# evroon/mav-detection

Measured on AMD Instinct MI355X. Metric: frame-pairs/sec at 1920x1080, higher is better.
Workload: dtype f32; 1 GPU; 1920x1080, batch 64 per GPU, Farneback + FoE + phi/threshold + box; global_batch=64, parallelism=frame-parallel x1, record_exchange=none (1 GPU), torch_in_process=False

## Files before the change

mav-detection_amd/csrc/kernels_flow.hip:

```cpp
#include "mavflow_internal.h"

#include <algorithm>
#include <type_traits>

static __device__ __forceinline__ int clampi(int v, int lo, int hi) { return v < lo ? lo : (v > hi ? hi : v); }

struct TileMap { int tiles_x, tiles_y, per_img, n_tiles, strip_w, xcd, ty0; };
static __device__ __forceinline__ bool tile_of_block(const TileMap& tm, int* s, int* tx, int* ty)
{
    const int per = ((int)gridDim.x + 7) >> 3;
    const int tile = tm.xcd ? (int)(blockIdx.x & 7) * per + (int)(blockIdx.x >> 3) : (int)blockIdx.x;
    if (tile >= tm.n_tiles) return false;
    const int img = tile / tm.per_img;
    int tr = tile - img * tm.per_img;
    const int strip_tiles = tm.strip_w * tm.tiles_y;
    const int st = tr / strip_tiles;
    tr -= st * strip_tiles;
    const int x_base = st * tm.strip_w;
    const int sw = min(tm.strip_w, tm.tiles_x - x_base);
    const int row = tr / sw;
    *s = img; *ty = row + tm.ty0; *tx = x_base + tr - row * sw;
    return true;
}
static TileMap make_tile_map(int w, int h, int G, int tile_w, int tile_h, int ty0 = 0, int ty1 = -1, int strip = 0)
// ... 758 lines not shown
    const int dword_ok = quad_ok(f);
    const int esize = (int)sizeof(T);
    if (f.G <= 8) return blur_multi_launch(st, f, dword_ok, jobs);
    bool done[MAV_MAX_JOBS] = {false};
    for (int i = 0; i < jobs.n; i++) {
        if (done[i]) continue;
        auto path_of = [&](const BlurJob& J) {
            if (J.w == f.W && J.h == f.H) return -1;
            const FusedPlan fp = fused_plan(f.W, f.H, J.w, J.h, J.bp, dword_ok, esize);
            return fused_path_of(J.bp, fp.pitch_w, dword_ok, esize);
        };
        const int p = path_of(jobs.j[i]);
        BlurJobs sub{0, 0, {}};
        for (int k = i; k < jobs.n; k++)
            if (!done[k] && path_of(jobs.j[k]) == p) { sub.j[sub.n++] = jobs.j[k]; done[k] = true; }
        blur_multi_launch(st, f, dword_ok, sub);
    }
}

template <typename T>
__global__ __launch_bounds__(256) void k_blur3(const T* __restrict__ img, const T* __restrict__ img2, int split,
                                               size_t img_stride, int W, int H, float* __restrict__ out, size_t out_stride)
{
    blur3_block(image_of(img, img2, split, img_stride, blockIdx.z), out + (size_t)blockIdx.z * out_stride, W, H, blockIdx.x, blockIdx.y);
}

template <typename T>
bool blur_resize_needs_tmp(const FrameRun<T>& f, const LayerTarget& t)
{
    return !blur3_fast_ok(f.runs(), t) && !blur_resize_is_fused(f.W, f.H, t.w, t.h, t.bp.ksize, (int)sizeof(T));
}
template <typename T>
void launch_blur_resize(hipStream_t st, const FrameRun<T>& frames, const LayerTarget& t, const BlurScratch& scratch)
{
    const FrameRun<T> f = frames.runs();
    const int G = f.G, W = f.W, H = f.H, w = t.w, h = t.h;
    const BlurParams& bp = t.bp;
    if (blur3_fast_ok(f, t)) {
        dim3 grid((W / 4 + 63) / 64, ((H + 3) / 4 + 3) / 4, G);
        hipLaunchKernelGGL(k_blur3<T>, grid, dim3(256), 0, st, f.img, f.img2, f.split, f.img_stride, W, H, t.out, t.out_stride);
        return;
    }
    const int dword_ok = quad_ok(f);
    const int esize = (int)sizeof(T);
    const int pitch_w = staged_pitch_words(W, w, bp.ksize);
    if (!scratch.two_pass && blur_resize_is_fused(W, H, w, h, bp.ksize, esize)) {
        const FusedPlan fp = fused_plan(W, H, w, h, bp, dword_ok, esize);
        const dim3 grid((w + 63) / 64, (h + fp.th - 1) / fp.th, G);
        with_fused_path<T>(fused_path_of(bp, fp.pitch_w, dword_ok, esize), [&](auto P) {
            if constexpr (decltype(P)::value != FP_ANY)
                hipLaunchKernelGGL((k_blur_resize_fused<T, decltype(P)::value>), grid, dim3(256), fp.lds, st, f.img, f.img2, f.split, f.img_stride,
                                   W, H, w, h, bp, t.out, t.out_stride, fp.rows, fp.pitch_w, dword_ok, fp.th);
        });
        return;
    }
    int rows_blk = 16;
    while (rows_blk > 4 && (size_t)rows_blk * pitch_w * 4 * esize > 48 * 1024) rows_blk >>= 1;
    if ((size_t)rows_blk * pitch_w * 4 * esize <= 48 * 1024)
    {
        const int gx = (w + 63) / 64, nby = (H + rows_blk - 1) / rows_blk;
        const int gy = nby;
        const size_t lds_h = (size_t)((rows_blk * pitch_w * esize + 1) & ~1) * 4 + (size_t)((bp.ksize + 4) & ~3) * 8;
        hipLaunchKernelGGL(k_blur_resize_h<T>, dim3(gx, gy, G), dim3(256), lds_h, st, f.img, f.img2, f.split, f.img_stride, W, H, w, bp,
                           scratch.tmp, scratch.stride, rows_blk, pitch_w, dword_ok);
    }
    else
        hipLaunchKernelGGL(k_blur_resize_h_direct<T>, dim3((w + 63) / 64, ((H + 3) / 4 + 3) / 4, G), dim3(256), 0, st, f.img, f.img2, f.split,
                           f.img_stride, W, H, w, bp, scratch.tmp, scratch.stride);
    hipLaunchKernelGGL(k_blur_resize_v, dim3((w + 63) / 64, (h + 3) / 4, G), dim3(256), 0, st, (const float*)scratch.tmp, scratch.stride, H, w,
                       h, bp, t.out, t.out_stride);
}
#define MAV_BLUR_DEPTH(T)                                                                                     \
    template bool blur_multi_ok<T>(const FrameRun<T>&, const LayerTarget&);                                   \
    template void launch_blur_multi<T>(hipStream_t, const FrameRun<T>&, BlurJobs);                            \
    template bool blur_resize_needs_tmp<T>(const FrameRun<T>&, const LayerTarget&);                           \
    template void launch_blur_resize<T>(hipStream_t, const FrameRun<T>&, const LayerTarget&, const BlurScratch&);
MAV_BLUR_DEPTH(uint8_t)
MAV_BLUR_DEPTH(uint16_t)
MAV_BLUR_DEPTH(float)
#undef MAV_BLUR_DEPTH

#define PX 64
#define PY 16
template <int N_T>
static __device__ __forceinline__ void polyexp_tile(const float* __restrict__ src, float* __restrict__ dst, int w, int h, const PolyCoef& pc,
                                                    int tile_x, int tile_y, float* __restrict__ smem)
{
    const int n = N_T > 0 ? N_T : pc.n;
    const int EX = PX + 2 * n, EY = PY + 2 * n;
    float* tile = smem;
    float* v0 = tile + EX * EY;
    float* v1 = v0 + PY * EX;
    float* v2 = v1 + PY * EX;
    const int tid = threadIdx.x;
    const int x0 = tile_x * PX, y0 = tile_y * PY;

    if constexpr (N_T > 0) {
        constexpr int TOT = (PX + 2 * N_T) * (PY + 2 * N_T), CNT = (TOT + 255) / 256;
        float v[CNT];
#pragma unroll
        for (int j = 0; j < CNT; j++) {
            const int i = tid + 256 * j;
            if (i < TOT) {
                const int ly = i / EX, lx = i - ly * EX;
                const int gx = clampi(x0 - n + lx, 0, w - 1), gy = clampi(y0 - n + ly, 0, h - 1);
                v[j] = src[(size_t)gy * w + gx];
            }
        }
#pragma unroll
        for (int j = 0; j < CNT; j++)
            if (tid + 256 * j < TOT) tile[tid + 256 * j] = v[j];
    } else {
        for (int i = tid; i < EX * EY; i += 256) {
            const int ly = i / EX, lx = i - ly * EX;
            const int gx = clampi(x0 - n + lx, 0, w - 1), gy = clampi(y0 - n + ly, 0, h - 1);
            tile[i] = src[(size_t)gy * w + gx];
        }
    }
    __syncthreads();
    for (int i = tid; i < PY * EX; i += 256) {
        const int ly = i / EX, lx = i - ly * EX;
        const float* c = tile + (ly + n) * EX + lx;
        float t0 = c[0] * pc.g[0], t1 = 0.f, t2 = 0.f;
#pragma unroll
        for (int k = 1; k <= n; k++) {
            const float a = c[-k * EX], b = c[k * EX];
            const float p = a + b;
            t0 = fmaf(pc.g[k], p, t0);
            t1 = fmaf(pc.xg[k], b - a, t1);
            t2 = fmaf(pc.xxg[k], p, t2);
        }
        v0[i] = t0; v1[i] = t1; v2[i] = t2;
    }
    __syncthreads();
    const size_t npx = (size_t)w * h;
    for (int i = tid; i < PY * PX; i += 256) {
        const int ly = i >> 6, lx = i & 63;
        const int gx = x0 + lx, gy = y0 + ly;
        if (gx >= w || gy >= h) continue;
        const float* p0 = v0 + ly * EX + lx + n;
        const float* p1 = v1 + ly * EX + lx + n;
        const float* p2 = v2 + ly * EX + lx + n;
        float b1 = p0[0] * pc.g[0], b2 = 0.f, b3 = p1[0] * pc.g[0], b4 = 0.f, b5 = p2[0] * pc.g[0], b6 = 0.f;
#pragma unroll
        for (int k = 1; k <= n; k++) {
            const float a0 = p0[-k], c0 = p0[k], a1 = p1[-k], c1 = p1[k], a2 = p2[-k], c2 = p2[k];
            const float tg = c0 + a0;
            b1 = fmaf(tg, pc.g[k], b1);
            b4 = fmaf(tg, pc.xxg[k], b4);
            b2 = fmaf(c0 - a0, pc.xg[k], b2);
            b3 = fmaf(c1 + a1, pc.g[k], b3);
            b6 = fmaf(c1 - a1, pc.xg[k], b6);
            b5 = fmaf(c2 + a2, pc.g[k], b5);
        }
        const size_t o = (size_t)gy * w + gx;
        dst[o] = b3 * pc.ig11;
        dst[npx + o] = b2 * pc.ig11;
        dst[2 * npx + o] = fmaf(b5, pc.ig33, b1 * pc.ig03);
        dst[3 * npx + o] = fmaf(b4, pc.ig33, b1 * pc.ig03);
        dst[4 * npx + o] = b6 * pc.ig55;
    }
}

template <int N_T>
__global__ __launch_bounds__(256) void k_polyexp(const float* __restrict__ I, size_t I_stride, int w, int h, PolyCoef pc, TileMap tm,
                                                 float* __restrict__ R, size_t R_stride)
{
    int img_s, tile_x, tile_y;
    if (!tile_of_block(tm, &img_s, &tile_x, &tile_y)) return;
    extern __shared__ __attribute__((aligned(16))) float smem[];
    polyexp_tile<N_T>(I + (size_t)img_s * I_stride, R + (size_t)img_s * R_stride, w, h, pc, tile_x, tile_y, smem);
}

template <int N_T>
__global__ __launch_bounds__(256) void k_polyexp_multi(PolyJobs jobs, PolyCoef pc)
{
    int k = 0;
    for (int i = 1; i < jobs.n; i++) k = (int)blockIdx.x >= jobs.j[i].first_block ? i : k;
    const PolyJob J = jobs.j[k];
    const int tile = (int)blockIdx.x - J.first_block;
    const int img_s = tile / J.per_img, rem = tile - img_s * J.per_img;
    const int tile_y = rem / J.tiles_x, tile_x = rem - tile_y * J.tiles_x;
    extern __shared__ __attribute__((aligned(16))) float smem[];
    polyexp_tile<N_T>(J.I + (size_t)img_s * J.I_stride, J.R + (size_t)img_s * J.R_stride, J.w, J.h, pc, tile_x, tile_y, smem);
}
void launch_polyexp_multi(hipStream_t st, PolyJobs jobs, int G, const PolyCoef& pc)
{
    const int n = pc.n;
    const size_t lds = sizeof(float) * ((size_t)(PX + 2 * n) * (PY + 2 * n) + 3 * (size_t)PY * (PX + 2 * n));
    int blocks = 0;
    for (int i = 0; i < jobs.n; i++) {
        PolyJob& J = jobs.j[i];
        J.tiles_x = (J.w + PX - 1) / PX;
        J.per_img = J.tiles_x * ((J.h + PY - 1) / PY);
        J.first_block = blocks;
        blocks += J.per_img * G;
    }
    if (n == 8) hipLaunchKernelGGL(k_polyexp_multi<8>, dim3(blocks), dim3(256), lds, st, jobs, pc);
    else if (n == 7) hipLaunchKernelGGL(k_polyexp_multi<7>, dim3(blocks), dim3(256), lds, st, jobs, pc);
    else if (n == 5) hipLaunchKernelGGL(k_polyexp_multi<5>, dim3(blocks), dim3(256), lds, st, jobs, pc);
    else hipLaunchKernelGGL(k_polyexp_multi<0>, dim3(blocks), dim3(256), lds, st, jobs, pc);
}

void launch_polyexp(hipStream_t st, const float* I, size_t I_stride, int G, int w, int h, const PolyCoef& pc, float* R,
                    size_t R_stride)
{
    const int n = pc.n;
    const size_t lds = sizeof(float) * ((size_t)(PX + 2 * n) * (PY + 2 * n) + 3 * (size_t)PY * (PX + 2 * n));
    TileMap tm = make_tile_map(w, h, G, PX, PY);
    tm.xcd = 0;
    const dim3 grid(tile_grid(tm));
    if (n == 8)
        hipLaunchKernelGGL(k_polyexp<8>, grid, dim3(256), lds, st, I, I_stride, w, h, pc, tm, R, R_stride);
    else if (n == 7)
        hipLaunchKernelGGL(k_polyexp<7>, grid, dim3(256), lds, st, I, I_stride, w, h, pc, tm, R, R_stride);
    else if (n == 5)
        hipLaunchKernelGGL(k_polyexp<5>, grid, dim3(256), lds, st, I, I_stride, w, h, pc, tm, R, R_stride);
    else
        hipLaunchKernelGGL(k_polyexp<0>, grid, dim3(256), lds, st, I, I_stride, w, h, pc, tm, R, R_stride);
}

struct GatherPx {
    float p00[5], p01[5], p10[5], p11[5];
    float fx, fy;
    bool inside;
};
static __device__ __forceinline__ void gather_issue(const float* __restrict__ R1p, size_t npx, int w, int h, int x, int y, float dx,
                                                    float dy, GatherPx& g)
{
    float fx = x + dx, fy = y + dy;
    const int x1 = (int)floorf(fx), y1 = (int)floorf(fy);
    g.fx = fx - x1; g.fy = fy - y1;
    g.inside = (unsigned)x1 < (unsigned)(w - 1) && (unsigned)y1 < (unsigned)(h - 1);
    const int xc = g.inside ? x1 : 0, yc = g.inside ? y1 : 0;
    const float* p = R1p + (size_t)yc * w + xc;
#pragma unroll
    for (int c = 0; c < 5; c++) {
        g.p00[c] = p[0]; g.p01[c] = p[1]; g.p10[c] = p[w]; g.p11[c] = p[w + 1];
        p += npx;
    }
}
static __device__ __forceinline__ void gather_inside(const float* __restrict__ R1p, size_t npx, int w, int h, int x, int y, float dx,
                                                     float dy, GatherPx& g)
{
    float fx = x + dx, fy = y + dy;
    const int x1 = (int)floorf(fx), y1 = (int)floorf(fy);
    g.fx = fx - x1; g.fy = fy - y1;
    g.inside = (unsigned)x1 < (unsigned)(w - 1) && (unsigned)y1 < (unsigned)(h - 1);
    if (!g.inside) return;
    const float* p = R1p + (size_t)y1 * w + x1;
#pragma unroll
    for (int c = 0; c < 5; c++) {
        g.p00[c] = p[0]; g.p01[c] = p[1]; g.p10[c] = p[w]; g.p11[c] = p[w + 1];
        p += npx;
    }
}
static __device__ __forceinline__ void update_finish(const float q[5], const GatherPx& g, int w, int h, int x, int y, float dx,
                                                     float dy, float out[5])
{
#pragma clang fp contract(off)
    float r2, r3, r4, r5, r6;
    if (g.inside) {
        const float gx = 1.f - g.fx, gy = 1.f - g.fy;
        const float a00 = gx * gy, a01 = g.fx * gy, a10 = gx * g.fy, a11 = g.fx * g.fy;
        r2 = fmaf(a11, g.p11[0], fmaf(a10, g.p10[0], fmaf(a01, g.p01[0], a00 * g.p00[0])));
        r3 = fmaf(a11, g.p11[1], fmaf(a10, g.p10[1], fmaf(a01, g.p01[1], a00 * g.p00[1])));
        r4 = fmaf(a11, g.p11[2], fmaf(a10, g.p10[2], fmaf(a01, g.p01[2], a00 * g.p00[2])));
        r5 = fmaf(a11, g.p11[3], fmaf(a10, g.p10[3], fmaf(a01, g.p01[3], a00 * g.p00[3])));
        r6 = fmaf(a11, g.p11[4], fmaf(a10, g.p10[4], fmaf(a01, g.p01[4], a00 * g.p00[4])));
        r4 = (q[2] + r4) * 0.5f;
        r5 = (q[3] + r5) * 0.5f;
        r6 = (q[4] + r6) * 0.25f;
    } else {
        r2 = r3 = 0.f;
        r4 = q[2]; r5 = q[3]; r6 = q[4] * 0.5f;
    }
    r2 = (q[0] - r2) * 0.5f;
    r3 = (q[1] - r3) * 0.5f;
    r2 += fmaf(r4, dy, r6 * dx);
    r3 += fmaf(r6, dy, r5 * dx);
    const int BORDER = 5;
    if ((unsigned)(x - BORDER) >= (unsigned)(w - BORDER * 2) || (unsigned)(y - BORDER) >= (unsigned)(h - BORDER * 2)) {
        auto bw = [](int d) { return d < 2 ? 0.14f : 0.4472f; };
        const float scale = (x < BORDER ? bw(x) : 1.f) * (x >= w - BORDER ? bw(w - x - 1) : 1.f) *
                            (y < BORDER ? bw(y) : 1.f) * (y >= h - BORDER ? bw(h - y - 1) : 1.f);
        r2 *= scale; r3 *= scale; r4 *= scale; r5 *= scale; r6 *= scale;
    }
    out[0] = fmaf(r4, r4, r6 * r6);
    out[1] = (r4 + r5) * r6;
    out[2] = fmaf(r5, r5, r6 * r6);
    out[3] = fmaf(r4, r2, r6 * r3);
    out[4] = fmaf(r6, r2, r5 * r3);
}

static __device__ __forceinline__ void update_px(const float* __restrict__ R0p, const float* __restrict__ R1p, size_t npx,
                                                 int w, int h, int x, int y, float dx, float dy, float* __restrict__ Mp)
{
    const size_t idx = (size_t)y * w + x;
    float q[5], o[5];
#pragma unroll
    for (int c = 0; c < 5; c++) q[c] = R0p[c * npx + idx];
    GatherPx g;
    gather_inside(R1p, npx, w, h, x, y, dx, dy, g);
    update_finish(q, g, w, h, x, y, dx, dy, o);
#pragma unroll
    for (int c = 0; c < 5; c++) Mp[c * npx + idx] = o[c];
}

static __device__ __forceinline__ void solve_px(float g11, float g12, float g22, float h1, float h2, float* u, float* v)
{
    const float p = g12 * g12, pe = fmaf(g12, g12, -p);
    const float det = (fmaf(g11, g22, -p) - pe) + 1e-3f;
    const float idet = 1.f / det;
    const float qa = g12 * h1, qae = fmaf(g12, h1, -qa);
    const float qb = g12 * h2, qbe = fmaf(g12, h2, -qb);
    *u = (fmaf(g11, h2, -qa) - qae) * idet;
    *v = (fmaf(g22, h1, -qb) - qbe) * idet;
}

static __device__ __forceinline__ float2 upsample_flow(const float* __restrict__ pf, int pw, int ph, float mul, double scale_x,
                                                       double scale_y, int x, int y)
{
#pragma clang fp contract(off)
    float fy = (float)((y + 0.5) * scale_y - 0.5);
    int sy = (int)floorf(fy);
    fy -= sy;
    if (sy < 0) { fy = 0.f; sy = 0; }
    if (sy >= ph - 1) { fy = 0.f; sy = ph - 1; }
    const int sy1 = sy + 1 < ph ? sy + 1 : sy;
    float fx = (float)((x + 0.5) * scale_x - 0.5);
    int sx = (int)floorf(fx);
    fx -= sx;
    if (sx < 0) { fx = 0.f; sx = 0; }
    if (sx >= pw - 1) { fx = 0.f; sx = pw - 1; }
    const int sx1 = sx + 1 < pw ? sx + 1 : sx;
    const float a0 = 1.f - fx, a1 = fx, b0 = 1.f - fy, b1 = fy;
    const float2 p00 = *(const float2*)(pf + ((size_t)sy * pw + sx) * 2);
    const float2 p01 = *(const float2*)(pf + ((size_t)sy * pw + sx1) * 2);
    const float2 p10 = *(const float2*)(pf + ((size_t)sy1 * pw + sx) * 2);
    const float2 p11 = *(const float2*)(pf + ((size_t)sy1 * pw + sx1) * 2);
    return make_float2(((p00.x * a0 + p01.x * a1) * b0 + (p10.x * a0 + p11.x * a1) * b1) * mul,
                       ((p00.y * a0 + p01.y * a1) * b0 + (p10.y * a0 + p11.y * a1) * b1) * mul);
}

template <int MODE>
__global__ __launch_bounds__(256) void k_update_matrices(const float* __restrict__ R0, const float* __restrict__ R1,
                                                         size_t R_stride, const float* __restrict__ fsrc, size_t f_stride,
                                                         int pw, int ph, float mul, double scale_x, double scale_y, int w,
                                                         int h, float* __restrict__ M, size_t M_stride, int y_begin, int y_end)
{
    const int x = blockIdx.x * 64 + (threadIdx.x & 63);
    const int y = y_begin + blockIdx.y * 4 + (threadIdx.x >> 6);
    if (x >= w || y >= y_end) return;
    const int s = blockIdx.z;
    float dx = 0.f, dy = 0.f;
    if (MODE == 1) {
        const float2 f = upsample_flow(fsrc + (size_t)s * f_stride, pw, ph, mul, scale_x, scale_y, x, y);
        dx = f.x; dy = f.y;
    } else if (MODE == 2) {
        const float2 f = *(const float2*)(fsrc + (size_t)s * f_stride + ((size_t)y * w + x) * 2);
        dx = f.x; dy = f.y;
    }
    update_px(R0 + (size_t)s * R_stride, R1 + (size_t)s * R_stride, (size_t)w * h, w, h, x, y, dx, dy,
              M + (size_t)s * M_stride);
}

void launch_initial_m(hipStream_t st, const InitialMArgs& a, const FlowSource& src)
{
    const int y_begin = a.y_begin < 0 ? 0 : a.y_begin, y_end = (a.y_end < 0 || a.y_end > a.h) ? a.h : a.y_end;
    if (y_end <= y_begin) return;
    const auto k = src.kind == FlowSource::COARSER ? k_update_matrices<1> : src.kind == FlowSource::FIELD ? k_update_matrices<2> : k_update_matrices<0>;
    hipLaunchKernelGGL(k, dim3((a.w + 63) / 64, (y_end - y_begin + 3) / 4, a.G), dim3(256), 0, st, a.R0, a.R1, a.R_stride, src.flow, src.stride,
                       src.pw, src.ph, src.mul, (double)src.pw / a.w, (double)src.ph / a.h, a.w, a.h, a.M, a.M_stride, y_begin, y_end);
}

struct BoxWindow {
    float scale;
    template <int M_T, int N, bool REGS, typename In, typename Out>
    __device__ __forceinline__ void sums(int m_rt, In in, Out out) const
    {
        const int win = 2 * (M_T > 0 ? M_T : m_rt) + 1;
        constexpr int UNROLL = REGS ? N : 8;
        decltype(in(0)) sum{};
#pragma unroll
        for (int k = 0; k < win; k++) sum += in(k);
#pragma unroll UNROLL
// ... 53 lines not shown
        }
    }
    __device__ __forceinline__ void solve(float g11, float g12, float g22, float h1, float h2, float* u, float* v) const
    {
        solve_gauss_px(g11, g12, g22, h1, h2, u, v);
    }
};

static inline void iter_geometry(int m, int* ext, int* pitch, int* plane)
{
    *ext = MAV_TILE + 2 * m;
    *pitch = (*ext & 1) ? *ext : *ext + 1;
    int p = *ext * *pitch;
    while ((p - *ext) % 32 != 0) p++;
    *plane = p;
}

size_t blur_iter_lds_bytes(int winsize)
{
    int ext, pitch, plane;
    iter_geometry(winsize / 2, &ext, &pitch, &plane);
    return sizeof(float) * 5 * (size_t)plane;
}

template <typename Win, int M_T>
__global__ __launch_bounds__(256) void k_blur_iter_generic(const float* __restrict__ M_in, float* __restrict__ M_out, size_t M_stride,
                                                   const float* __restrict__ R0, const float* __restrict__ R1, size_t R_stride,
                                                   int w, int h, int m_rt, int pitch, int plane, Win win, int do_update,
                                                   float* __restrict__ flow, size_t f_stride)
{
    extern __shared__ __attribute__((aligned(16))) float lds[];
    const int m = M_T > 0 ? M_T : m_rt;
    const int ext = MAV_TILE + 2 * m;
    const int tid = threadIdx.x;
    const int s = blockIdx.z;
    const int x0 = blockIdx.x * MAV_TILE, y0 = blockIdx.y * MAV_TILE;
    const size_t npx = (size_t)w * h;
    const float* Min = M_in + (size_t)s * M_stride;

    for (int c = 0; c < 5; c++) {
        const float* P = Min + c * npx;
        float* L = lds + c * plane;
        for (int i = tid; i < ext * ext; i += 256) {
            const int ly = i / ext, lx = i - ly * ext;
            const int gx = clampi(x0 - m + lx, 0, w - 1), gy = clampi(y0 - m + ly, 0, h - 1);
            L[ly * pitch + lx] = P[(size_t)gy * w + gx];
        }
    }
    __syncthreads();
    for (int t = tid; t < 5 * ext; t += 256) {
        const int c = t / ext, lx = t - c * ext;
        float* col = lds + c * plane + lx;
        win.template sums<M_T, MAV_TILE, false>(m, [&](int i) { return col[i * pitch]; }, [&](int y, float a) { col[y * pitch] = a; });
    }
    __syncthreads();
    for (int t = tid; t < 5 * MAV_TILE; t += 256) {
        const int c = t >> 5, y = t & 31;
        float* row = lds + c * plane + y * pitch;
        win.template sums<M_T, MAV_TILE, false>(m, [&](int i) { return row[i]; }, [&](int x, float a) { row[x] = a; });
    }
    __syncthreads();
    const float* R0p = R0 + (size_t)s * R_stride;
    const float* R1p = R1 + (size_t)s * R_stride;
    float* Mo = M_out + (size_t)s * M_stride;
    float* fo = flow + (size_t)s * f_stride;
    const int lx = tid & 31;
    const int gx = x0 + lx;
#pragma unroll
    for (int j = 0; j < 4; j++) {
        const int ly = (tid >> 5) + 8 * j;
        const int gy = y0 + ly;
        if (gx >= w || gy >= h) continue;
        const float* L = lds + ly * pitch + lx;
        float u, v;
        win.solve(L[0], L[plane], L[2 * plane], L[3 * plane], L[4 * plane], &u, &v);
        *(float2*)(fo + ((size_t)gy * w + gx) * 2) = make_float2(u, v);
        if (do_update) update_px(R0p, R1p, npx, w, h, gx, gy, u, v, Mo);
    }
}

#define FT_X 64
#define FT_Y 16

struct __attribute__((packed, aligned(4))) F2U { float x, y; };
template <typename Win, int M_T, bool AL, bool WT>
__global__ __launch_bounds__(256) void k_blur_iter_fast(const float* __restrict__ M_in, float* __restrict__ M_out,
                                                        size_t M_stride, const float* __restrict__ R0,
                                                        const float* __restrict__ R1, size_t R_stride, int w, int h,
                                                        TileMap tm, Win win,
                                                        int do_update, int store_flow, float* __restrict__ flow, size_t f_stride)
{
    constexpr int EXT_X = FT_X + 2 * M_T;
    constexpr int EXT_Y = FT_Y + 2 * M_T;
    constexpr int PITCH = (EXT_X + 3) & ~3;
    constexpr int PLANE = FT_Y * PITCH + (EXT_X - (FT_Y * PITCH) % 32 + 64) % 32;
    static_assert(PLANE % 4 == 0 && EXT_X % 2 == 0, "plane must keep 16-byte alignment");
    __shared__ __attribute__((aligned(16))) float vs[5 * PLANE];
    const int tid = threadIdx.x;
    const int lane = tid & 63, wv = tid >> 6;
    int s, tx, ty;
    if (!tile_of_block(tm, &s, &tx, &ty)) return;
    const int x0 = tx * FT_X, y0 = ty * FT_Y;
    const size_t npx = (size_t)w * h;
    const float* Min = M_in + (size_t)s * M_stride;
    const float* R0p = R0 + (size_t)s * R_stride;
    const float* R1p = R1 + (size_t)s * R_stride;

    STAMP(ts0);
    float q[4][5];
    int gys[4];
    const int gxc = min(x0 + lane, w - 1);
    if (do_update) {
#pragma unroll
        for (int j = 0; j < 4; j++) {
            gys[j] = min(y0 + wv * 4 + j, h - 1);
            const size_t idx = (size_t)gys[j] * w + gxc;
#pragma unroll
            for (int c = 0; c < 5; c++) q[j][c] = R0p[c * npx + idx];
        }
    }

    if (x0 >= M_T && x0 + FT_X + M_T <= w) {
        constexpr int NP = EXT_X / 2;
        for (int t = tid; t < 5 * NP; t += 256) {
            const int c = t / NP, pr = t - c * NP;
            const float* col = Min + c * npx + (x0 - M_T + 2 * pr);
            float2 v[EXT_Y];
#pragma unroll
            for (int i = 0; i < EXT_Y; i++) {
                const float* pp = col + (size_t)clampi(y0 - M_T + i, 0, h - 1) * w;
                if (AL) v[i] = *(const float2*)pp;
                else { const F2U t = *(const F2U*)pp; v[i] = make_float2(t.x, t.y); }
            }
            float* out = vs + c * PLANE + 2 * pr;
            win.template sums<M_T, FT_Y, true>(M_T, [&](int i) { return v[i]; }, [&](int y, float2 a) { *(float2*)(out + y * PITCH) = a; });
        }
    } else {
        for (int t = tid; t < 5 * EXT_X; t += 256) {
            const int c = t / EXT_X, lx = t - c * EXT_X;
            const int gx = clampi(x0 - M_T + lx, 0, w - 1);
            const float* col = Min + c * npx + gx;
            float v[EXT_Y];
#pragma unroll
            for (int i = 0; i < EXT_Y; i++) v[i] = col[(size_t)clampi(y0 - M_T + i, 0, h - 1) * w];
            float* out = vs + c * PLANE + lx;
            win.template sums<M_T, FT_Y, true>(M_T, [&](int i) { return v[i]; }, [&](int y, float a) { out[y * PITCH] = a; });
        }
    }
    STAMP(ts1);
    __syncthreads();
    STAMP(ts2);

    {
        const int quad = (lane & 31) >> 2;
        const int grp = (lane >> 5) * 2 + ((quad == 1 || quad == 2 || quad == 4 || quad == 7) ? 1 : 0);
        const int qpos = (quad == 0 || quad == 1) ? 0 : ((quad == 3 || quad == 2) ? 1 : ((quad == 5 || quad == 4) ? 2 : 3));
        const int pos = qpos * 4 + (lane & 3);
        const int ly = wv * 4 + grp;
        const int lx0 = pos * 4;
        const int gx = x0 + lx0, gy = y0 + ly;
        float S[5][4];
#pragma unroll
        for (int c = 0; c < 5; c++) {
            const float4* p = (const float4*)(vs + c * PLANE + ly * PITCH + lx0);
            constexpr int NV = (4 + 2 * M_T + 3) / 4;
            float f[4 * NV];
#pragma unroll
            for (int k = 0; k < NV; k++) {
                const float4 t4 = p[k];
                f[4 * k] = t4.x; f[4 * k + 1] = t4.y; f[4 * k + 2] = t4.z; f[4 * k + 3] = t4.w;
            }
            win.template sums<M_T, 4, true>(M_T, [&](int i) { return f[i]; }, [&](int j, float a) { S[c][j] = a; });
        }
        float u[4], v[4];
#pragma unroll
        for (int j = 0; j < 4; j++) win.solve(S[0][j], S[1][j], S[2][j], S[3][j], S[4][j], &u[j], &v[j]);
        if (store_flow && gx < w && gy < h) {
            float* fo = flow + (size_t)s * f_stride + ((size_t)gy * w + gx) * 2;
            if (AL) {
                *(float4*)fo = make_float4(u[0], v[0], u[1], v[1]);
                *(float4*)(fo + 4) = make_float4(u[2], v[2], u[3], v[3]);
            } else {
#pragma unroll
                for (int j = 0; j < 4; j++)
                    if (gx + j < w) *(float2*)(fo + 2 * j) = make_float2(u[j], v[j]);
            }
        }
        if (!do_update) return;
        *(float4*)(vs + ly * PITCH + lx0) = make_float4(u[0], u[1], u[2], u[3]);
        *(float4*)(vs + PLANE + ly * PITCH + lx0) = make_float4(v[0], v[1], v[2], v[3]);
    }
    __builtin_amdgcn_fence(__ATOMIC_RELEASE, "wavefront");
    __builtin_amdgcn_wave_barrier();
    __builtin_amdgcn_fence(__ATOMIC_ACQUIRE, "wavefront");
    STAMP(ts3);

    float* Mo = M_out + (size_t)s * M_stride;
    const bool colok = x0 + lane < w;
#pragma unroll
    for (int jb = 0; jb < 4; jb += 2) {
        GatherPx g[2];
        float fu[2], fv[2];
#pragma unroll
        for (int jj = 0; jj < 2; jj++) {
            const int ly = wv * 4 + jb + jj;
            fu[jj] = vs[ly * PITCH + lane];
            fv[jj] = vs[PLANE + ly * PITCH + lane];
            gather_issue(R1p, npx, w, h, gxc, gys[jb + jj], fu[jj], fv[jj], g[jj]);
        }
#pragma unroll
        for (int jj = 0; jj < 2; jj++) {
            float o[5];
            update_finish(q[jb + jj], g[jj], w, h, gxc, gys[jb + jj], fu[jj], fv[jj], o);
            if (colok && y0 + wv * 4 + jb + jj < h) {
                const size_t idx = (size_t)gys[jb + jj] * w + gxc;
#pragma unroll
                for (int c = 0; c < 5; c++) {
                    if constexpr (WT) __hip_atomic_store((unsigned*)(Mo + c * npx + idx), __float_as_uint(o[c]), __ATOMIC_RELAXED, __HIP_MEMORY_SCOPE_AGENT);
                    else Mo[c * npx + idx] = o[c];
                }
            }
        }
#ifdef MAV_STAMPS
        if (jb == 0) { STAMP(tsm); STAMP_ADD(3, ts3, tsm); STAMP_ADD(5, tsm, tsm); }
#endif
    }
    STAMP(ts4);
    STAMP_ADD(0, ts0, ts1); STAMP_ADD(1, ts1, ts2); STAMP_ADD(2, ts2, ts3); STAMP_ADD(4, ts3, ts4); STAMP_ADD(6, ts0, ts4); STAMP_ADD(7, 0ull, 1ull);
}

static bool aligned16(const void* p) { return ((uintptr_t)p & 15) == 0; }
int blur_iter_tile_rows(int h) { return (h + FT_Y - 1) / FT_Y; }
static bool blur_iter_vec_ok(const SweepArgs& a)
{
    return (a.w % 4 == 0) && (a.M_stride % 4 == 0) && (a.R_stride % 4 == 0) && (a.f_stride % 4 == 0) && aligned16(a.M_in) && aligned16(a.M_out) &&
           aligned16(a.R0) && aligned16(a.R1) && aligned16(a.flow);
}
bool blur_iter_bands_ok(const SweepArgs& a) { return a.winsize / 2 == 6 && blur_iter_vec_ok(a); }

template <typename Win, bool AL>
static void launch_sweep_fast(hipStream_t st, const TileMap& tm, const SweepArgs& a, const Win& win)
{
    const bool wt = a.write_through && a.do_update;
    const auto k = wt ? k_blur_iter_fast<Win, 6, AL, true> : k_blur_iter_fast<Win, 6, AL, false>;
    hipLaunchKernelGGL(k, dim3(tile_grid(tm)), dim3(256), 0, st, a.M_in, a.M_out, a.M_stride, a.R0, a.R1, a.R_stride, a.w, a.h, tm, win,
                       a.do_update, a.store_flow, a.flow, a.f_stride);
}

template <typename Win>
static void launch_sweep(hipStream_t st, const SweepArgs& a, const Win& win)
{
    const int m = a.winsize / 2;
    if (m == 6 && blur_iter_vec_ok(a)) {
        const TileMap tm = make_tile_map(a.w, a.h, a.G, FT_X, FT_Y, a.ty0, a.ty1, a.strip);
        if (tm.n_tiles == 0) return;
        return launch_sweep_fast<Win, true>(st, tm, a, win);
    }
    if (m == 6 && a.f_stride % 2 == 0 && ((uintptr_t)a.flow & 7) == 0)
        return launch_sweep_fast<Win, false>(st, make_tile_map(a.w, a.h, a.G, FT_X, FT_Y, 0, -1, a.strip), a, win);
    int ext, pitch, plane;
    iter_geometry(m, &ext, &pitch, &plane);
    const size_t lds = sizeof(float) * 5 * (size_t)plane;
    const dim3 grid((a.w + MAV_TILE - 1) / MAV_TILE, (a.h + MAV_TILE - 1) / MAV_TILE, a.G);
    const auto k = m == 6 ? k_blur_iter_generic<Win, 6> : k_blur_iter_generic<Win, 0>;
    hipLaunchKernelGGL(k, grid, dim3(256), lds, st, a.M_in, a.M_out, a.M_stride, a.R0, a.R1, a.R_stride, a.w, a.h, m, pitch, plane, win,
                       a.do_update, a.flow, a.f_stride);
}

void launch_blur_iter(hipStream_t st, const SweepArgs& a)
{
    if (a.gauss) launch_sweep(st, a, GaussWindow{*a.gauss});
    else launch_sweep(st, a, BoxWindow{(float)(1.0 / ((double)a.winsize * a.winsize))});
}

const char* blur_iter_prepare(int winsize)
{
    const size_t lds = blur_iter_lds_bytes(winsize);
    if (lds <= (size_t)64 * 1024) return nullptr;
    hipError_t e = hipFuncSetAttribute((const void*)k_blur_iter_generic<BoxWindow, 0>, hipFuncAttributeMaxDynamicSharedMemorySize, (int)lds);
    if (e == hipSuccess) e = hipFuncSetAttribute((const void*)k_blur_iter_generic<GaussWindow, 0>, hipFuncAttributeMaxDynamicSharedMemorySize, (int)lds);
    return e == hipSuccess ? nullptr : hipGetErrorString(e);
}

__global__ __launch_bounds__(256) void k_probe_r3w1(const float4* __restrict__ a, const float4* __restrict__ b, const float4* __restrict__ c,
                                                    float4* __restrict__ d, size_t n)
{
    for (size_t i = (size_t)blockIdx.x * 256 + threadIdx.x; i < n; i += (size_t)gridDim.x * 256) {
        const float4 x = a[i], y = b[i], z = c[i];
        d[i] = make_float4(x.x + y.x + z.x, x.y + y.y + z.y, x.z + y.z + z.z, x.w + y.w + z.w);
    }
}
// ... 5 lines not shown
```

mav-detection_amd/csrc/mavflow.cpp:

```cpp
#include <assert.h>
#include <dlfcn.h>
#include <math.h>
#include <float.h>
#include <stdarg.h>
#include <stdio.h>
#include <stdlib.h>
#include <string.h>

#include <algorithm>
#include <atomic>
#include <condition_variable>
#include <deque>
#include <map>
#include <mutex>
#include <string>
#include <thread>
#include <vector>

#include "mavflow_internal.h"
#include "../../include/mavflow_truth.h"
#include "../../include/mavflow_validation.h"

static thread_local std::string g_err;
static int fail(int code, const char* fmt, ...)
// ... 3350 lines not shown
    ProcessArgs a;
    a.flow_in = flow; a.samples = samples; a.omega = omega; a.dt = dt; a.frame0 = frame0; a.sky = sky; a.foe_par = fp; a.thr = tp;
    a.phi = phi; a.mask_fixed = mask_fixed; a.mask_dyn = mask_dyn; a.results = results;
    return process_host(c, "mav_detect", batch, a);
}

extern "C" int mav_stage_phi_mask(mav_ctx* c, const float* flow, const double* foe, const double* omega, const double* dt,
                                  const uint8_t* sky, int batch, const mav_thr_params* tp, double* phi, uint8_t* mask_fixed,
                                  uint8_t* mask_dyn, int32_t* box)
{
    HostCall h(c, "mav_stage_phi_mask");
    CHK(h.fresh(batch));
    if (!flow || !foe) return fail(MAV_ERR_ARG, "mav_stage_phi_mask: NULL argument");
    const size_t n = c->n0 * batch;
    const mav_thr_params t = thr_or_defaults(tp);
    DetectArgs a;
    a.flow32 = h.in(flow, n * 2 * sizeof(float));
    a.foe_in = h.in(foe, sizeof(double) * 2 * batch);
    a.sky = h.in(sky, n);
    a.phi = h.out(phi, n * sizeof(double));
    a.mask_fixed = h.out(mask_fixed, n);
    a.mask_dyn = h.out(mask_dyn, n);
    a.box_out = h.out(box, sizeof(int32_t) * 4 * batch);
    a.thr = &t;
    CHK(h.staged());
    CHK(upload_derot(c, omega, dt, nullptr, batch, true, &a.derot));
    CHK(detect_dev(c, batch, a));
    return h.finish();
}

extern "C" int mav_stage_coefficients(mav_ctx* c, int k, float* g, float* xg, float* xxg, float* ig, float* blur_taps)
{
    if (!c) return fail(MAV_ERR_ARG, "mav_stage_coefficients: NULL context");
    const int n = c->pc.n;
    for (int i = 0; i <= n; i++) {
        if (g) g[i] = c->pc.g[i];
        if (xg) xg[i] = c->pc.xg[i];
        if (xxg) xxg[i] = c->pc.xxg[i];
    }
    if (ig) { ig[0] = c->pc.ig11; ig[1] = c->pc.ig03; ig[2] = c->pc.ig33; ig[3] = c->pc.ig55; }
    if (blur_taps) {
        HostCall h(c, "mav_stage_coefficients");
        const Layer* l;
        CHK(h.fresh_layer(k, &l));
        HIPCHK(hipMemcpy(blur_taps, l->g, sizeof(float) * l->ksize, hipMemcpyDeviceToHost));
    }
    return MAV_OK;
}

static int stage_blur_resize(mav_ctx* c, const void* img, int depth, int k, bool two_pass, float* out)
{
    if (c && !depth_esize(depth)) return fail(MAV_ERR_ARG, "mav_stage_blur_resize_ex: depth %d is none of MAV_DEPTH_8U / 16U / 32F", depth);
    HostCall h(c, "mav_stage_blur_resize");
    const Layer* l;
    CHK(h.fresh_layer(k, &l));
    if (!img || !out) return fail(MAV_ERR_ARG, "mav_stage_blur_resize: NULL argument");
    const size_t n = (size_t)l->w * l->h;
    const void* di = h.in(img, c->n0 * depth_esize(depth));
    float* dout = h.out(out, n * sizeof(float));
    float* dtmp = h.scratch<float>(c->htmp_stride * sizeof(float));
    CHK(h.staged());
    with_depth(depth, [&](auto* px) {
        typedef std::remove_const_t<std::remove_pointer_t<decltype(px)>> T;
        launch_blur_resize(c->stream, FrameRun<T>{(const T*)di, nullptr, 0, c->n0, 1, c->W, c->H}, {dout, n, blur_of(c, *l), l->w, l->h},
                           {dtmp, c->htmp_stride, two_pass});
    });
    CHK(check_launch("blur_resize"));
    return h.finish();
}
extern "C" int mav_stage_blur_resize(mav_ctx* c, const uint8_t* img, int k, float* out) { return stage_blur_resize(c, img, MAV_DEPTH_8U, k, false, out); }
extern "C" int mav_stage_blur_resize_two_pass(mav_ctx* c, const uint8_t* img, int k, float* out) { return stage_blur_resize(c, img, MAV_DEPTH_8U, k, true, out); }
extern "C" int mav_stage_blur_resize_ex(mav_ctx* c, const void* img, int depth, int k, int two_pass, float* out)
{
    return stage_blur_resize(c, img, depth, k, two_pass != 0, out);
}
extern "C" int mav_stage_polyexp(mav_ctx* c, const float* I, int k, float* R)
{
    HostCall h(c, "mav_stage_polyexp");
    const Layer* l;
    CHK(h.fresh_layer(k, &l));
    if (!I || !R) return fail(MAV_ERR_ARG, "mav_stage_polyexp: NULL argument");
    const size_t n = (size_t)l->w * l->h;
    const float* di = h.in(I, n * sizeof(float));
    float* dr = h.out(R, 5 * n * sizeof(float));
    CHK(h.staged());
    launch_polyexp(c->stream, di, n, 1, l->w, l->h, c->pc, dr, 5 * n);
    CHK(check_launch("polyexp"));
    return h.finish();
}
extern "C" int mav_stage_update_matrices(mav_ctx* c, const float* R0, const float* R1, const float* flow, int k, float* M)
{
    HostCall h(c, "mav_stage_update_matrices");
    const Layer* l;
    CHK(h.fresh_layer(k, &l));
    if (!R0 || !R1 || !flow || !M) return fail(MAV_ERR_ARG, "mav_stage_update_matrices: NULL argument");
    const size_t n = (size_t)l->w * l->h;
    const float* d0 = h.in(R0, 5 * n * sizeof(float));
    const float* d1 = h.in(R1, 5 * n * sizeof(float));
    const float* df = h.in(flow, 2 * n * sizeof(float));
    float* dm = h.out(M, 5 * n * sizeof(float));
    CHK(h.staged());
    launch_initial_m(c->stream, {{d0, d1, 5 * n, 1, l->w, l->h}, dm, 5 * n}, FlowSource::field(df, 2 * n));
    CHK(check_launch("update_matrices"));
    return h.finish();
}
extern "C" int mav_stage_update_matrices_from(mav_ctx* c, const float* R0, const float* R1, const float* flow_coarse, int k, float* M)
{
    HostCall h(c, "mav_stage_update_matrices_from");
    const Layer* l;
    CHK(h.fresh_layer(k, &l));
    if (!R0 || !R1 || !M) return fail(MAV_ERR_ARG, "mav_stage_update_matrices_from: NULL argument");
    if (flow_coarse && k + 1 >= (int)c->layers.size())
        return fail(MAV_ERR_ARG, "mav_stage_update_matrices_from: layer %d is the top layer, it has no coarser flow", k);
    const size_t n = (size_t)l->w * l->h;
    const size_t nc = flow_coarse ? (size_t)c->layers[k + 1].w * c->layers[k + 1].h : 0;
    const float* d0 = h.in(R0, 5 * n * sizeof(float));
    const float* d1 = h.in(R1, 5 * n * sizeof(float));
    const float* df = h.in(flow_coarse, 2 * nc * sizeof(float));
    float* dm = h.out(M, 5 * n * sizeof(float));
    CHK(h.staged());
    launch_initial_m(c->stream, {{d0, d1, 5 * n, 1, l->w, l->h}, dm, 5 * n}, flow_coarse ? coarser_flow(c, k + 1, df, 2 * nc) : FlowSource{});
    CHK(check_launch("update_matrices"));
    return h.finish();
}
extern "C" int mav_stage_initial_flow(mav_ctx* c, const float* flow0, int k, float* out)
{
    HostCall h(c, "mav_stage_initial_flow");
    const Layer* l;
    CHK(h.fresh_layer(k, &l));
    if (!flow0 || !out) return fail(MAV_ERR_ARG, "mav_stage_initial_flow: NULL argument");
    const size_t n = (size_t)l->w * l->h;
    double scale = 1;
    for (int i = 0; i < k; i++) scale *= c->fb.pyr_scale;
    const float* di = h.in(flow0, 2 * c->n0 * sizeof(float));
    float* dout = h.out(out, 2 * n * sizeof(float));
    CHK(h.staged());
    launch_area_resize_flow(c->stream, di, 2 * c->n0, c->W, c->H, dout, 2 * n, l->w, l->h, 1, scale);
    CHK(check_launch("area_resize_flow"));
    return h.finish();
}
extern "C" int mav_stage_blur_iter(mav_ctx* c, const float* R0, const float* R1, const float* M, int k, int update, float* flow, float* M_out)
{
    HostCall h(c, "mav_stage_blur_iter");
    const Layer* l;
    CHK(h.fresh_layer(k, &l));
    if (!R0 || !R1 || !M || !flow || (update && !M_out)) return fail(MAV_ERR_ARG, "mav_stage_blur_iter: NULL argument");
    const size_t n = (size_t)l->w * l->h;
    const float* d0 = h.in(R0, 5 * n * sizeof(float));
    const float* d1 = h.in(R1, 5 * n * sizeof(float));
    const float* dm = h.in(M, 5 * n * sizeof(float));
    float* dmo = h.scratch<float>(5 * n * sizeof(float));
    float* df = h.out(flow, 2 * n * sizeof(float));
    h.fetch(update ? M_out : nullptr, dmo, 5 * n * sizeof(float));
    CHK(h.staged());
    SweepArgs a{{d0, d1, 5 * n, 1, l->w, l->h}, dm, dmo, 5 * n, c->fb.winsize, df, 2 * n, update, 1};
    a.strip = c->strip; a.gauss = window_taps(c);
    launch_blur_iter(c->stream, a);
    CHK(check_launch("blur_iter"));
    return h.finish();
}

typedef int (*nccl_get_uid_t)(void*);
struct uid128 { char b[128]; };
typedef int (*nccl_init_rank2_t)(void**, int, uid128, int);
typedef int (*nccl_destroy_t)(void*);
typedef int (*nccl_allgather_t)(const void*, void*, size_t, int, void*, hipStream_t);
typedef const char* (*nccl_errstr_t)(int);
static void* g_rccl = nullptr;
static int rccl_sym(const char* name, void** fn)
{
    if (!g_rccl) {
        g_rccl = dlopen("librccl.so.1", RTLD_NOW | RTLD_GLOBAL);
        if (!g_rccl) g_rccl = dlopen("librccl.so", RTLD_NOW | RTLD_GLOBAL);
        if (!g_rccl) return fail(MAV_ERR_STATE, "cannot load RCCL: %s", dlerror());
    }
    *fn = dlsym(g_rccl, name);
    if (!*fn) return fail(MAV_ERR_STATE, "RCCL symbol %s missing", name);
    return MAV_OK;
}
typedef int (*nccl_get_version_t)(int*);
extern "C" int mav_runtime_info(char* buf, size_t cap)
{
    if (!buf || cap < 16) return fail(MAV_ERR_ARG, "mav_runtime_info: NULL argument");
    int rt = 0, drv = 0, nccl = 0;
    if (hipRuntimeGetVersion(&rt) != hipSuccess) rt = -1;
    if (hipDriverGetVersion(&drv) != hipSuccess) drv = -1;
    void* fn = nullptr;
    if (g_rccl && (fn = dlsym(g_rccl, "ncclGetVersion"))) ((nccl_get_version_t)fn)(&nccl);
    snprintf(buf, cap, "{\"built_with_hip\": \"%d.%d.%d\", \"hip_runtime\": %d, \"hip_runtime_major\": %d, \"hip_driver\": %d, \"rccl\": %d}",
             HIP_VERSION_MAJOR, HIP_VERSION_MINOR, HIP_VERSION_PATCH, rt, rt > 0 ? rt / 10000000 : -1, drv, nccl);
    return MAV_OK;
}
extern "C" int mav_comm_unique_id(void* id128)
{
    if (!id128) return fail(MAV_ERR_ARG, "mav_comm_unique_id: NULL");
    void* fn;
    CHK(rccl_sym("ncclGetUniqueId", &fn));
    int rc = ((nccl_get_uid_t)fn)(id128);
    return rc ? fail(MAV_ERR_HIP, "ncclGetUniqueId failed: %d", rc) : MAV_OK;
}
extern "C" int mav_comm_init(mav_ctx* c, const void* id128, int rank, int nranks, void** comm_out)
{
    if (!c || !id128 || !comm_out) return fail(MAV_ERR_ARG, "mav_comm_init: NULL argument");
    HIPCHK(hipSetDevice(c->device));
    int rt = 0;
    HIPCHK(hipRuntimeGetVersion(&rt));
    if (rt / 10000000 != HIP_VERSION_MAJOR)
        return fail(MAV_ERR_STATE, "mav_comm_init: libmavflow was built with HIP %d.%d but the process runs HIP runtime %d (major %d): rebuild against "
                    "the runtime the launcher loads", HIP_VERSION_MAJOR, HIP_VERSION_MINOR, rt, rt / 10000000);
    void* fn;
    CHK(rccl_sym("ncclCommInitRank", &fn));
    uid128 id;
    memcpy(&id, id128, sizeof(id));
    int rc = ((nccl_init_rank2_t)fn)(comm_out, nranks, id, rank);
    return rc ? fail(MAV_ERR_HIP, "ncclCommInitRank failed: %d", rc) : MAV_OK;
}
typedef int (*nccl_comm_count_t)(void*, int*);
extern "C" int mav_comm_count(void* comm, int* nranks)
{
    if (!comm || !nranks) return fail(MAV_ERR_ARG, "mav_comm_count: NULL argument");
    void* fn;
    CHK(rccl_sym("ncclCommCount", &fn));
    int rc = ((nccl_comm_count_t)fn)(comm, nranks);
    return rc ? fail(MAV_ERR_HIP, "ncclCommCount failed: %d", rc) : MAV_OK;
}
extern "C" int mav_comm_destroy(void* comm)
{
    if (!comm) return MAV_OK;
    void* fn;
    CHK(rccl_sym("ncclCommDestroy", &fn));
    ((nccl_destroy_t)fn)(comm);
    return MAV_OK;
// ... 1326 lines not shown
```

mav-detection_amd/csrc/mavflow_internal.h:

```cpp
#pragma once
#include <hip/hip_runtime.h>
#include <stdint.h>

#include "../../include/mavflow.h"

#define MAV_MAX_POLY_N 16
#define MAV_TILE 32

struct PolyCoef {
    int n;
    float g[MAV_MAX_POLY_N + 1], xg[MAV_MAX_POLY_N + 1], xxg[MAV_MAX_POLY_N + 1];
    float ig11, ig03, ig33, ig55;
};

struct BlurParams {
    int ksize;
    int fixed3;
    const float* g;
    double scale_x;
    double scale_y;
    const int* xs; const float* xf;
    const int* ys; const float* yf;
};

enum { MAV_PAIR_PROMOTE = 0, MAV_PAIR_DEROTATE = 1, MAV_PAIR_FRAME0 = 2 };
struct DerotParams {
    double o0, o1, o2, sx, sy;
    int mode;
};

static __device__ __forceinline__ void derot_apply(float2 f, const DerotParams* __restrict__ dp, int W, int H, int row, int col,
                                                   double* fu, double* fv)
{
    double u = (double)f.x, v = (double)f.y;
    if (dp && dp->mode == MAV_PAIR_DEROTATE) {
        const double x = -((double)col / (double)W - 0.5) * 2.0;
        const double y = -((double)row / (double)H - 0.5) * 2.0;
        const double o0 = dp->o0, o1 = dp->o1, o2 = dp->o2;
        double du = (((o0 * x) * y - o1 * (x * x)) - o1) + o2 * y;
        double dv = ((((-o2) * x + o0) + o0 * (y * y))) - (o1 * x) * y;
        du = du * dp->sx;
        dv = dv * dp->sy;
        u = u - du;
        v = v - dv;
    }
    *fu = u; *fv = v;
}
static __device__ __forceinline__ void derot_apply(double2 f, const DerotParams*, int, int, int, int, double* fu, double* fv)
{
    *fu = f.x; *fv = f.y;
}

#define MAV_MAX_JOBS 6
struct PolyJob { const float* I; float* R; size_t I_stride, R_stride; int w, h, tiles_x, per_img, first_block, pad; };
struct PolyJobs { int n, pad; PolyJob j[MAV_MAX_JOBS]; };

template <typename T>
struct FrameRun {
    const T *img, *img2;
    int split;
    size_t img_stride;
    int G, W, H;
    FrameRun runs() const { return img2 ? *this : FrameRun{img, img, G, img_stride, G, W, H}; }
};
struct LayerTarget { float* out; size_t out_stride; BlurParams bp; int w, h; };
struct BlurJob : LayerTarget { int fused, gx, gy, first_block, rows_cap, pitch_w, th, pad; };
struct BlurJobs { int n, pad; BlurJob j[MAV_MAX_JOBS]; };
struct BlurScratch { float* tmp; size_t stride; bool two_pass = false; };
template <typename T>
void launch_blur_resize(hipStream_t st, const FrameRun<T>& f, const LayerTarget& t, const BlurScratch& scratch);
bool blur_resize_is_fused(int W, int H, int w, int h, int ksize, int esize = 1);
template <typename T>
bool blur_resize_needs_tmp(const FrameRun<T>& f, const LayerTarget& t);
void launch_polyexp(hipStream_t st, const float* I, size_t I_stride, int G, int w, int h, const PolyCoef& pc, float* R,
                    size_t R_stride);
void launch_polyexp_multi(hipStream_t st, PolyJobs jobs, int G, const PolyCoef& pc);
template <typename T>
bool blur_multi_ok(const FrameRun<T>& f, const LayerTarget& t);
template <typename T>
void launch_blur_multi(hipStream_t st, const FrameRun<T>& f, BlurJobs jobs);

struct PairOperands { const float *R0, *R1; size_t R_stride; int G, w, h; };
struct FlowSource {
    enum Kind { ZERO = 0, COARSER = 1, FIELD = 2 };
    Kind kind = ZERO;
    const float* flow = nullptr;
    size_t stride = 0;
    int pw = 0, ph = 0;
    float mul = 0.f;
    static FlowSource coarser(const float* flow, size_t stride, int pw, int ph, float mul)
    {
        return flow ? FlowSource{COARSER, flow, stride, pw, ph, mul} : FlowSource{};
    }
    static FlowSource field(const float* flow, size_t stride) { return FlowSource{FIELD, flow, stride}; }
    FlowSource from_pair(int s0) const { FlowSource u = *this; if (u.flow) u.flow += (size_t)s0 * stride; return u; }
};
struct InitialMArgs : PairOperands {
    float* M;
    size_t M_stride;
    int y_begin = 0, y_end = -1;
};
void launch_initial_m(hipStream_t st, const InitialMArgs& a, const FlowSource& src);
#define MAV_MAX_WIN_HALF 32
struct GaussTaps { float k[MAV_MAX_WIN_HALF + 1]; };
void gauss_taps(int winsize, GaussTaps* out);
struct SweepArgs : PairOperands {
    const float* M_in;
    float* M_out;
    size_t M_stride;
    int winsize;
    float* flow;
    size_t f_stride;
    int do_update, store_flow;
    int ty0 = 0, ty1 = -1;
    int strip = 0;
    bool write_through = false;
    const GaussTaps* gauss = nullptr;
};
void launch_blur_iter(hipStream_t st, const SweepArgs& a);
int blur_iter_tile_rows(int h);
bool blur_iter_bands_ok(const SweepArgs& a);
size_t blur_iter_lds_bytes(int winsize);
const char* blur_iter_prepare(int winsize);

void launch_probe_r3w1(hipStream_t st, const float* a, const float* b, const float* c, float* d, size_t n_float4);

struct FoeScratch {
    double* cand;
    int* count;
    unsigned long long* best_key;
    unsigned* done;
};
void launch_foe_f32(hipStream_t st, const float* flow, const DerotParams* derot , const uint32_t* samples,
                    int B, int W, int H, int N, double mag2_thr, float mag2_thr_f32 , double dist2_thr,
                    FoeScratch s, double* foe, int32_t* box_acc ,
                    unsigned long long* max_phi_bits );
void launch_foe_f64(hipStream_t st, const double* flow, const uint32_t* samples, int B, int W, int H, int N, double mag2_thr,
                    double dist2_thr, FoeScratch s, double* foe, int32_t* box_acc, unsigned long long* max_phi_bits);
void launch_box_init(hipStream_t st, int32_t* box_acc, unsigned long long* max_phi_bits, unsigned* done , int B);
struct PhiLaunch {
    unsigned* done = nullptr;
    mav_result* results = nullptr;
    int32_t* box_out = nullptr;
    bool screen = true;
    int yloop = 0;
};
void launch_phi_mask_f32(hipStream_t st, const float* flow, const DerotParams* derot, const double* foe, const uint8_t* sky,
                         int B, int W, int H, mav_thr_params thr, double* phi, uint8_t* mask_fixed, uint8_t* mask_dyn,
                         int32_t* box_acc, unsigned long long* max_phi_bits, const PhiLaunch& pl);
void launch_phi_mask_f64(hipStream_t st, const double* flow, const double* foe, const uint8_t* sky, int B, int W, int H,
                         mav_thr_params thr, double* phi, uint8_t* mask_fixed, uint8_t* mask_dyn, int32_t* box_acc,
                         unsigned long long* max_phi_bits, const PhiLaunch& pl);
void launch_box_finalize(hipStream_t st, const int32_t* box_acc, int B, int32_t* box);
void launch_derotate(hipStream_t st, const float* flow, const DerotParams* derot, int B, int W, int H, double* out);
void launch_bbox_u8(hipStream_t st, const uint8_t* img, int B, int W, int H, int* maxv , int32_t* box_acc);
void launch_window_max(hipStream_t st, const uint8_t* img, int B, int W, int H, unsigned long long* key ,
                       int64_t* out);
void launch_tpr_fpr(hipStream_t st, const uint8_t* gt, const uint8_t* mask, unsigned mask_value, int B, int W, int H,
                    unsigned long long* counts );
void launch_tpr_fpr2(hipStream_t st, const uint8_t* gt, size_t gt_stride, const uint8_t* mask0, const uint8_t* mask1, unsigned mask_value, int B,
                     int W, int H, unsigned long long* counts0 , unsigned long long* counts1 );
struct RocThr {
    int ka, km;
    double mag0_sq_lo;
    double ang[MAV_ROC_MAX_ANGLES], mag[MAV_ROC_MAX_MAGS];
// ... 198 lines not shown
```

Before: 2695 frame-pairs/s.

## Store polynomial expansion interleaved per pixel for contiguous gathers

```diff
diff --git a/mav-detection_amd/csrc/kernels_flow.hip b/mav-detection_amd/csrc/kernels_flow.hip
--- a/mav-detection_amd/csrc/kernels_flow.hip
+++ b/mav-detection_amd/csrc/kernels_flow.hip
@@ -864,6 +864,18 @@
 
 #define PX 64
 #define PY 16
+struct __attribute__((packed, aligned(4))) F2U { float x, y; };
+struct __attribute__((packed, aligned(4))) F4U { float x, y, z, w; };
+static __device__ __forceinline__ void load5(const float* __restrict__ p, float v[5])
+{
+    const F4U a = *(const F4U*)p;
+    v[0] = a.x; v[1] = a.y; v[2] = a.z; v[3] = a.w; v[4] = p[4];
+}
+static __device__ __forceinline__ void store5(float* __restrict__ p, const float v[5])
+{
+    *(F4U*)p = F4U{v[0], v[1], v[2], v[3]};
+    p[4] = v[4];
+}
 template <int N_T>
 static __device__ __forceinline__ void polyexp_tile(const float* __restrict__ src, float* __restrict__ dst, int w, int h, const PolyCoef& pc,
                                                     int tile_x, int tile_y, float* __restrict__ smem)
@@ -915,7 +927,6 @@
         v0[i] = t0; v1[i] = t1; v2[i] = t2;
     }
     __syncthreads();
-    const size_t npx = (size_t)w * h;
     for (int i = tid; i < PY * PX; i += 256) {
         const int ly = i >> 6, lx = i & 63;
         const int gx = x0 + lx, gy = y0 + ly;
@@ -935,12 +946,8 @@
             b6 = fmaf(c1 - a1, pc.xg[k], b6);
             b5 = fmaf(c2 + a2, pc.g[k], b5);
         }
-        const size_t o = (size_t)gy * w + gx;
-        dst[o] = b3 * pc.ig11;
-        dst[npx + o] = b2 * pc.ig11;
-        dst[2 * npx + o] = fmaf(b5, pc.ig33, b1 * pc.ig03);
-        dst[3 * npx + o] = fmaf(b4, pc.ig33, b1 * pc.ig03);
-        dst[4 * npx + o] = b6 * pc.ig55;
+        const float r[5] = {b3 * pc.ig11, b2 * pc.ig11, fmaf(b5, pc.ig33, b1 * pc.ig03), fmaf(b4, pc.ig33, b1 * pc.ig03), b6 * pc.ig55};
+        store5(dst + 5 * ((size_t)gy * w + gx), r);
     }
 }
 
@@ -1007,35 +1014,35 @@
     float fx, fy;
     bool inside;
 };
-static __device__ __forceinline__ void gather_issue(const float* __restrict__ R1p, size_t npx, int w, int h, int x, int y, float dx,
-                                                    float dy, GatherPx& g)
+static __device__ __forceinline__ void gather_row(const float* __restrict__ p, float a[5], float b[5])
+{
+    const F4U t0 = *(const F4U*)p, t1 = *(const F4U*)(p + 4);
+    const F2U t2 = *(const F2U*)(p + 8);
+    a[0] = t0.x; a[1] = t0.y; a[2] = t0.z; a[3] = t0.w; a[4] = t1.x;
+    b[0] = t1.y; b[1] = t1.z; b[2] = t1.w; b[3] = t2.x; b[4] = t2.y;
+}
+static __device__ __forceinline__ void gather_issue(const float* __restrict__ R1p, int w, int h, int x, int y, float dx, float dy, GatherPx& g)
 {
     float fx = x + dx, fy = y + dy;
     const int x1 = (int)floorf(fx), y1 = (int)floorf(fy);
     g.fx = fx - x1; g.fy = fy - y1;
     g.inside = (unsigned)x1 < (unsigned)(w - 1) && (unsigned)y1 < (unsigned)(h - 1);
     const int xc = g.inside ? x1 : 0, yc = g.inside ? y1 : 0;
-    const float* p = R1p + (size_t)yc * w + xc;
-#pragma unroll
-    for (int c = 0; c < 5; c++) {
-        g.p00[c] = p[0]; g.p01[c] = p[1]; g.p10[c] = p[w]; g.p11[c] = p[w + 1];
-        p += npx;
-    }
-}
-static __device__ __forceinline__ void gather_inside(const float* __restrict__ R1p, size_t npx, int w, int h, int x, int y, float dx,
-                                                     float dy, GatherPx& g)
+    const float* p = R1p + 5 * ((size_t)yc * w + xc);
+    const size_t row = (w > 1 && h > 1) ? 5 * (size_t)w : 0;
+    gather_row(p, g.p00, g.p01);
+    gather_row(p + row, g.p10, g.p11);
+}
+static __device__ __forceinline__ void gather_inside(const float* __restrict__ R1p, int w, int h, int x, int y, float dx, float dy, GatherPx& g)
 {
     float fx = x + dx, fy = y + dy;
     const int x1 = (int)floorf(fx), y1 = (int)floorf(fy);
     g.fx = fx - x1; g.fy = fy - y1;
     g.inside = (unsigned)x1 < (unsigned)(w - 1) && (unsigned)y1 < (unsigned)(h - 1);
     if (!g.inside) return;
-    const float* p = R1p + (size_t)y1 * w + x1;
-#pragma unroll
-    for (int c = 0; c < 5; c++) {
-        g.p00[c] = p[0]; g.p01[c] = p[1]; g.p10[c] = p[w]; g.p11[c] = p[w + 1];
-        p += npx;
-    }
+    const float* p = R1p + 5 * ((size_t)y1 * w + x1);
+    gather_row(p, g.p00, g.p01);
+    gather_row(p + 5 * (size_t)w, g.p10, g.p11);
 }
 static __device__ __forceinline__ void update_finish(const float q[5], const GatherPx& g, int w, int h, int x, int y, float dx,
                                                      float dy, float out[5])
@@ -1080,10 +1087,9 @@
 {
     const size_t idx = (size_t)y * w + x;
     float q[5], o[5];
-#pragma unroll
-    for (int c = 0; c < 5; c++) q[c] = R0p[c * npx + idx];
+    load5(R0p + 5 * idx, q);
     GatherPx g;
-    gather_inside(R1p, npx, w, h, x, y, dx, dy, g);
+    gather_inside(R1p, w, h, x, y, dx, dy, g);
     update_finish(q, g, w, h, x, y, dx, dy, o);
 #pragma unroll
     for (int c = 0; c < 5; c++) Mp[c * npx + idx] = o[c];
@@ -1303,7 +1309,6 @@
 #define FT_X 64
 #define FT_Y 16
 
-struct __attribute__((packed, aligned(4))) F2U { float x, y; };
 template <typename Win, int M_T, bool AL, bool WT>
 __global__ __launch_bounds__(256) void k_blur_iter_fast(const float* __restrict__ M_in, float* __restrict__ M_out,
                                                         size_t M_stride, const float* __restrict__ R0,
@@ -1335,9 +1340,7 @@
 #pragma unroll
         for (int j = 0; j < 4; j++) {
             gys[j] = min(y0 + wv * 4 + j, h - 1);
-            const size_t idx = (size_t)gys[j] * w + gxc;
-#pragma unroll
-            for (int c = 0; c < 5; c++) q[j][c] = R0p[c * npx + idx];
+            load5(R0p + 5 * ((size_t)gys[j] * w + gxc), q[j]);
         }
     }
 
@@ -1427,7 +1430,7 @@
             const int ly = wv * 4 + jb + jj;
             fu[jj] = vs[ly * PITCH + lane];
             fv[jj] = vs[PLANE + ly * PITCH + lane];
-            gather_issue(R1p, npx, w, h, gxc, gys[jb + jj], fu[jj], fv[jj], g[jj]);
+            gather_issue(R1p, w, h, gxc, gys[jb + jj], fu[jj], fv[jj], g[jj]);
         }
 #pragma unroll
         for (int jj = 0; jj < 2; jj++) {
diff --git a/mav-detection_amd/csrc/mavflow.cpp b/mav-detection_amd/csrc/mavflow.cpp
--- a/mav-detection_amd/csrc/mavflow.cpp
+++ b/mav-detection_amd/csrc/mavflow.cpp
@@ -3456,11 +3456,11 @@
     if (!I || !R) return fail(MAV_ERR_ARG, "mav_stage_polyexp: NULL argument");
     const size_t n = (size_t)l->w * l->h;
     const float* di = h.in(I, n * sizeof(float));
-    float* dr = h.out(R, 5 * n * sizeof(float));
+    std::vector<float> e(5 * n); float* dr = h.out(e.data(), 5 * n * sizeof(float));
     CHK(h.staged());
     launch_polyexp(c->stream, di, n, 1, l->w, l->h, c->pc, dr, 5 * n);
     CHK(check_launch("polyexp"));
-    return h.finish();
+    return planes_of_expansion(h.finish(), e, n, R);
 }
 extern "C" int mav_stage_update_matrices(mav_ctx* c, const float* R0, const float* R1, const float* flow, int k, float* M)
 {
@@ -3469,8 +3469,8 @@
     CHK(h.fresh_layer(k, &l));
     if (!R0 || !R1 || !flow || !M) return fail(MAV_ERR_ARG, "mav_stage_update_matrices: NULL argument");
     const size_t n = (size_t)l->w * l->h;
-    const float* d0 = h.in(R0, 5 * n * sizeof(float));
-    const float* d1 = h.in(R1, 5 * n * sizeof(float));
+    const std::vector<float> e0 = expansion_of_planes(R0, n), e1 = expansion_of_planes(R1, n);
+    const float *d0 = h.in(e0.data(), 5 * n * sizeof(float)), *d1 = h.in(e1.data(), 5 * n * sizeof(float));
     const float* df = h.in(flow, 2 * n * sizeof(float));
     float* dm = h.out(M, 5 * n * sizeof(float));
     CHK(h.staged());
@@ -3488,8 +3488,8 @@
         return fail(MAV_ERR_ARG, "mav_stage_update_matrices_from: layer %d is the top layer, it has no coarser flow", k);
     const size_t n = (size_t)l->w * l->h;
     const size_t nc = flow_coarse ? (size_t)c->layers[k + 1].w * c->layers[k + 1].h : 0;
-    const float* d0 = h.in(R0, 5 * n * sizeof(float));
-    const float* d1 = h.in(R1, 5 * n * sizeof(float));
+    const std::vector<float> e0 = expansion_of_planes(R0, n), e1 = expansion_of_planes(R1, n);
+    const float *d0 = h.in(e0.data(), 5 * n * sizeof(float)), *d1 = h.in(e1.data(), 5 * n * sizeof(float));
     const float* df = h.in(flow_coarse, 2 * nc * sizeof(float));
     float* dm = h.out(M, 5 * n * sizeof(float));
     CHK(h.staged());
@@ -3520,8 +3520,8 @@
     CHK(h.fresh_layer(k, &l));
     if (!R0 || !R1 || !M || !flow || (update && !M_out)) return fail(MAV_ERR_ARG, "mav_stage_blur_iter: NULL argument");
     const size_t n = (size_t)l->w * l->h;
-    const float* d0 = h.in(R0, 5 * n * sizeof(float));
-    const float* d1 = h.in(R1, 5 * n * sizeof(float));
+    const std::vector<float> e0 = expansion_of_planes(R0, n), e1 = expansion_of_planes(R1, n);
+    const float *d0 = h.in(e0.data(), 5 * n * sizeof(float)), *d1 = h.in(e1.data(), 5 * n * sizeof(float));
     const float* dm = h.in(M, 5 * n * sizeof(float));
     float* dmo = h.scratch<float>(5 * n * sizeof(float));
     float* df = h.out(flow, 2 * n * sizeof(float));
diff --git a/mav-detection_amd/csrc/mavflow_internal.h b/mav-detection_amd/csrc/mavflow_internal.h
--- a/mav-detection_amd/csrc/mavflow_internal.h
+++ b/mav-detection_amd/csrc/mavflow_internal.h
@@ -1,6 +1,7 @@
 #pragma once
 #include <hip/hip_runtime.h>
 #include <stdint.h>
+#include <vector>
 
 #include "../../include/mavflow.h"
 
@@ -81,6 +82,19 @@
 void launch_blur_multi(hipStream_t st, const FrameRun<T>& f, BlurJobs jobs);
 
 struct PairOperands { const float *R0, *R1; size_t R_stride; int G, w, h; };
+inline std::vector<float> expansion_of_planes(const float* planes, size_t n)
+{
+    std::vector<float> e(planes ? 5 * n : 0);
+    for (size_t c = 0; c < 5 && planes; c++)
+        for (size_t i = 0; i < n; i++) e[5 * i + c] = planes[c * n + i];
+    return e;
+}
+inline int planes_of_expansion(int rc, const std::vector<float>& e, size_t n, float* planes)
+{
+    for (size_t c = 0; c < 5 && rc == MAV_OK; c++)
+        for (size_t i = 0; i < n; i++) planes[c * n + i] = e[5 * i + c];
+    return rc;
+}
 struct FlowSource {
     enum Kind { ZERO = 0, COARSER = 1, FIELD = 2 };
     Kind kind = ZERO;
```

Result: faster. 2875 frame-pairs/s (median of 6 runs) (+6.7%).
